# Wangshihu12/colmap-pcd

Measured on AMD Instinct MI355X. Metric: NN queries/sec + BA-iter ms, 10M-pt cloud / 1M 3D feats, higher is better.
Workload: dtype f32 (NN distances) / f64 (association, BA); 1 GPU; M: 10000000-pt 'planes' cloud / 1000000 queries + BA scene 1000 cams / 1000000 pts / 4721253 obs / 900000 lidar terms (OPENCV), the same total at every N; cloud_points=10000000, queries=1000000, queries_this_rank=1000000, parallelism=single GPU

## Files before the change

### colmap-pcd_amd/csrc/nn.hip

```cpp
#include <atomic>
#include <cfloat>

#include "cloud.h"
#include "grid.h"
#include "prim.h"
#include "scratch.h"

namespace pcd {

void free_query_scratch(QueryScratch* s) { delete s; }

constexpr uint64_t kKeyInit = (uint64_t)0x7F7FFFFFu << 32;
constexpr uint64_t kSmallBatch = 65536;

struct BrickParams {
  int B, R;
  int Bx;
  int nb[3];
  uint32_t nbricks;
};

constexpr int kBrickCells = 2, kBrickCellsX = 2, kBrickHalo = 2;

static BrickParams make_bricks(const GridParams& g) {
// ... 542 lines not shown
  const uint32_t n = *count_ptr;
  const uint32_t e0 = (blockIdx.x * kFbcThreads + tid) * kFbcPer;
  if (blockIdx.x * kFbcThreads * kFbcPer >= n) return;
  uint32_t v[kFbcPer], cnt = 0;
  if (e0 + kFbcPer <= n) {
    const uint4 q = *reinterpret_cast<const uint4*>(list + e0);
    v[0] = q.x; v[1] = q.y; v[2] = q.z; v[3] = q.w;
  } else {
#pragma unroll
    for (uint32_t k = 0; k < kFbcPer; ++k) v[k] = e0 + k < n ? list[e0 + k] : 0xFFFFFFFFu;
  }
#pragma unroll
  for (uint32_t k = 0; k < kFbcPer; ++k) cnt += v[k] != 0xFFFFFFFFu ? 1u : 0u;
  const uint32_t inc = wave_scan_add_u32(cnt);
  if (lane == 63) s_wave[wave] = inc;
  __syncthreads();
  uint32_t before = 0, total = 0;
  for (uint32_t w = 0; w < kFbcThreads / 64; ++w) { before += w < wave ? s_wave[w] : 0u; total += s_wave[w]; }
  if (tid == 0) s_base = total ? atomicAdd(dense_count, total) : 0u;
  __syncthreads();
  uint32_t pos = s_base + before + inc - cnt;
#pragma unroll
  for (uint32_t k = 0; k < kFbcPer; ++k)
    if (v[k] != 0xFFFFFFFFu) dense[pos++] = v[k];
}

struct FbFused {
  const double* q;
  const double* max_range;
  uint64_t mr_count;
  double fixed_range;
};

template <int FUSED>
__global__ __launch_bounds__(256) void k_nn_fallback(GridParams g, PyramidParams py, const float4* __restrict__ sorted,
                                                      const uint32_t* __restrict__ cell_start,
                                                      const float* __restrict__ aabb,
                                                      const float4* __restrict__ seeds,
                                                      const float4* __restrict__ qf4,
                                                      const uint32_t* __restrict__ list,
                                                      const uint32_t* __restrict__ count_ptr, uint32_t count_imm,
                                                      uint64_t* __restrict__ keys, NnCounters* __restrict__ ctr,
                                                      int collect_stats, FbFused fu) {
  constexpr int kStack = kMaxPyrLevels - 2;
  __shared__ float s_lb[4][kStack][64];
  __shared__ uint32_t s_rng[4][kStack][64];
  __shared__ unsigned long long s_mask[4][kStack];
  const int lane = threadIdx.x & 63;
  const int wave = __builtin_amdgcn_readfirstlane((int)(threadIdx.x >> 6));
  const uint32_t count = count_ptr ? *count_ptr : count_imm;
  const uint32_t nwaves = gridDim.x * 4;
  const int top = py.nlev - 1;
  unsigned long long st_pts = 0, st_q = 0, st_steps = 0, st_leaves = 0;
  uint32_t st_max_steps = 0, st_max_leaves = 0;
  for (uint32_t e = blockIdx.x * 4 + wave; e < count; e += nwaves) {
    const uint32_t qi = list ? list[e] : e;
    float qx, qy, qz;
    uint64_t best;
    if (FUSED == 0) {
      const float4 q = qf4[qi];
      if (q.w == 0.f) continue;
      qx = q.x; qy = q.y; qz = q.z;
      best = keys[qi];
    } else {
      qx = (float)fu.q[3 * (size_t)qi]; qy = (float)fu.q[3 * (size_t)qi + 1]; qz = (float)fu.q[3 * (size_t)qi + 2];
      if (!(isfinite(qx) && isfinite(qy) && isfinite(qz))) {
        if (lane == 0) keys[qi] = PCD_KEY_NONE;
        continue;
      }
      best = FUSED == 2 ? bounded_init_key(fu.max_range ? fu.max_range[fu.mr_count == 1 ? 0 : qi] : fu.fixed_range,
                                             fu.q[3 * (size_t)qi], fu.q[3 * (size_t)qi + 1], fu.q[3 * (size_t)qi + 2])
                          : kKeyInit;
    }
    {
      const int sx = cell_coord(qx, g.origin[0], g.inv_h, g.dims[0]) >> 3;
      const int sy = cell_coord(qy, g.origin[1], g.inv_h, g.dims[1]) >> 3;
      const int sz = cell_coord(qz, g.origin[2], g.inv_h, g.dims[2]) >> 3;
      const float4 sp = seeds[((size_t)sz * py.seed_dims[1] + sy) * py.seed_dims[0] + sx];
      const uint64_t sk = make_key(l2_simple3(qx, qy, qz, sp.x, sp.y, sp.z), __float_as_uint(sp.w));
      best = sk < best ? sk : best;
    }
    double lane_best = __builtin_bit_cast(double, best);
    float best_d = __uint_as_float((uint32_t)(best >> 32));
    int lev = top;
    float cur_lb;
    unsigned long long cur_m;
    uint32_t rs = 0, rn = 0;
    uint32_t q_steps = 0, q_leaves = 0;
#define PCD_FB_EXPAND(cf, cn)                                                                                         \
    {                                                                                                                 \
      const uint32_t cn_ = (cn);                                                                                      \
      const uint32_t last = cn_ ? cn_ - 1u : 0u;                   \
      const uint32_t id = (cf) + ((uint32_t)lane < last ? (uint32_t)lane : last);                                     \
      const float4 lo = *reinterpret_cast<const float4*>(aabb + 8 * (size_t)id);             \
      const float4 hi = *reinterpret_cast<const float4*>(aabb + 8 * (size_t)id + 4);       \
           \
                      \
      const float px = __builtin_amdgcn_fmed3f(qx, lo.x, lo.w), pyc = __builtin_amdgcn_fmed3f(qy, lo.y, hi.x),        \
                  pz = __builtin_amdgcn_fmed3f(qz, lo.z, hi.y);                                                       \
      const float lbv = l2_simple3(qx, qy, qz, px, pyc, pz);                                                          \
      cur_lb = (uint32_t)lane < cn_ ? lbv : INFINITY;                                                                 \
      rs = __float_as_uint(hi.z); rn = __float_as_uint(hi.w);                                                         \
      cur_m = __ballot(cur_lb <= best_d);                                                                             \
    }
    PCD_FB_EXPAND(py.root_first, py.root_count);
    while (true) {
      ++q_steps;
      unsigned long long m = cur_m & __ballot(cur_lb <= best_d);
      if (m == 0) {
        if (lev == top) break;
        ++lev;
        cur_lb = s_lb[wave][lev - 2][lane];
        const uint32_t pr = s_rng[wave][lev - 2][lane];
        rs = pr & (kMaxPyrRecords - 1u); rn = (pr >> 26) + 1u;
        const unsigned long long pm = s_mask[wave][lev - 2];
        cur_m = ((unsigned long long)(uint32_t)__builtin_amdgcn_readfirstlane((int)(pm >> 32)) << 32) |
                (uint32_t)__builtin_amdgcn_readfirstlane((int)pm);
        continue;
      }
      const int sl = wave_argmin_u32(__float_as_uint(cur_lb), m);
      m &= ~(1ull << sl);
      cur_m = m;
      if (lev == 1) {
        const uint32_t s0 = (uint32_t)__builtin_amdgcn_readlane((int)rs, sl), n0 = (uint32_t)__builtin_amdgcn_readlane((int)rn, sl);
        for (uint32_t base = 0; base < n0; base += 128) {
          float4 p[2];
#pragma unroll
          for (int k = 0; k < 2; ++k) {
            const uint32_t gi = base + k * 64 + lane;
            p[k] = sorted[s0 + (gi < n0 ? gi : n0 - 1)];
          }
#pragma unroll
          for (int k = 0; k < 2; ++k) {
            const float d = l2_simple3(qx, qy, qz, p[k].x, p[k].y, p[k].z);
            lane_best = min_key_f64(lane_best, __builtin_bit_cast(double, make_key(d, __float_as_uint(p[k].w))));
          }
        }
        st_pts += n0;
        ++q_leaves;
        best = wave_min_u64(__builtin_bit_cast(uint64_t, lane_best));
        best_d = __uint_as_float((uint32_t)(best >> 32));
        unsigned long long mb = m & __ballot(cur_lb <= best_d);
        if (mb) {
          cur_m = m & ~mb;
          while (mb) {
            uint32_t a[4], c[4];
            uint32_t cmax = 0;
#pragma unroll
            for (int k = 0; k < 4; ++k) {
              const int r = mb ? __ffsll((long long)mb) - 1 : -1;
              mb &= mb - 1;
              a[k] = r >= 0 ? (uint32_t)__builtin_amdgcn_readlane((int)rs, r) : a[0];
              c[k] = r >= 0 ? (uint32_t)__builtin_amdgcn_readlane((int)rn, r) : 0u;
              cmax = c[k] > cmax ? c[k] : cmax;
              st_pts += c[k];
              q_leaves += r >= 0 ? 1 : 0;
            }
            for (uint32_t base = 0; base < cmax; base += 64) {
              float4 p[4];
              const uint32_t gi = base + lane;
#pragma unroll
              for (int k = 0; k < 4; ++k) p[k] = sorted[a[k] + (gi < c[k] ? gi : (c[k] ? c[k] - 1 : 0u))];
#pragma unroll
              for (int k = 0; k < 4; ++k) {
                const float d = l2_simple3(qx, qy, qz, p[k].x, p[k].y, p[k].z);
                lane_best = min_key_f64(lane_best, __builtin_bit_cast(double, make_key(d, __float_as_uint(p[k].w))));
              }
            }
          }
          best = wave_min_u64(__builtin_bit_cast(uint64_t, lane_best));
          best_d = __uint_as_float((uint32_t)(best >> 32));
        }
      } else {
        s_lb[wave][lev - 2][lane] = cur_lb;
        s_rng[wave][lev - 2][lane] = rs | ((rn - 1u) << 26);
        if (lane == 0) s_mask[wave][lev - 2] = cur_m;
        const uint32_t cf = (uint32_t)__builtin_amdgcn_readlane((int)rs, sl), cn = (uint32_t)__builtin_amdgcn_readlane((int)rn, sl);
        --lev;
        PCD_FB_EXPAND(cf, cn);
      }
    }
#undef PCD_FB_EXPAND
    if (lane == 0) keys[qi] = finalized_key(best);
    st_q += 1;
    st_steps += q_steps; st_leaves += q_leaves;
    st_max_steps = q_steps > st_max_steps ? q_steps : st_max_steps;
    st_max_leaves = q_leaves > st_max_leaves ? q_leaves : st_max_leaves;
  }
  if (collect_stats) {
    __shared__ unsigned long long s_st[4];
    __shared__ unsigned int s_mx[2];
    if (threadIdx.x < 4) s_st[threadIdx.x] = 0;
    if (threadIdx.x < 2) s_mx[threadIdx.x] = 0;
    __syncthreads();
    if (lane == 0) {
      atomicAdd(&s_st[0], st_pts); atomicAdd(&s_st[1], st_q); atomicAdd(&s_st[2], st_steps); atomicAdd(&s_st[3], st_leaves);
      atomicMax(&s_mx[0], st_max_steps); atomicMax(&s_mx[1], st_max_leaves);
    }
    __syncthreads();
    if (threadIdx.x == 0 && s_st[1]) {
      atomicAdd(&ctr->fallback_points, s_st[0]);
      atomicAdd(&ctr->pair_evals, s_st[0]);
      atomicAdd(&ctr->fallback_queries, s_st[1]);
      atomicAdd(&ctr->fb_steps, s_st[2]); atomicAdd(&ctr->fb_leaves, s_st[3]);
      atomicMax(&ctr->fb_max_steps, s_mx[0]); atomicMax(&ctr->fb_max_leaves, s_mx[1]);
    }
  }
}

constexpr unsigned g_fb_max_blocks = 16384;
struct FbQueries {
  const float4* qf4;
  FbFused fused;
  const uint32_t *list, *list_count;
};
template <int FUSED>
static void launch_fallback(const pcd_cloud* c, const float4* seeds, const FbQueries& src, uint64_t n, uint64_t* keys,
                            NnCounters* ctr, int collect_stats, hipStream_t s) {
  hipLaunchKernelGGL(k_nn_fallback<FUSED>, dim3((unsigned)std::min<uint64_t>(div_up(n, 4), g_fb_max_blocks)), dim3(256), 0,
                     s, c->grid, c->pyr, c->sorted.p, c->cell_start.p, c->blk_aabb.p, seeds, src.qf4, src.list,
                     src.list_count, src.list_count ? 0u : (uint32_t)n, keys, ctr, collect_stats, src.fused);
}
static std::atomic<int> g_collect_stats{0};
#ifdef PCD_ABLATE
static const int g_brick_blocks_per_cu = std::getenv("PCD_BRICK_BLOCKS") ? std::atoi(std::getenv("PCD_BRICK_BLOCKS")) : PCD_BRICK_MINWAVES;
#else
constexpr int g_brick_blocks_per_cu = PCD_BRICK_MINWAVES;
#endif
static std::atomic<int> g_nn_kernel{0};
static std::atomic<int> g_bk_sort{0};
static std::atomic<int> g_nn_schedule{0};

static pcd_status brick_slots(pcd_cloud* c, QueryScratch* sc, const BrickParams& b, hipStream_t s) {
  if (sc->bk_slot.p && sc->bk_nslots == b.nbricks) return PCD_OK;
  PCD_TRY(sc->bk_slot.reserve((size_t)b.nbricks / 32 + 1));
  DevBuf<uint32_t> flag;
  PCD_TRY(flag.reserve((size_t)b.nbricks + 1));
  hipLaunchKernelGGL(k_brick_occupied, dim3(div_up(b.nbricks, 256)), dim3(256), 0, s, c->grid, b, c->cell_start.p, flag.p);
  hipLaunchKernelGGL(k_brick_bitmap, dim3(div_up(div_up(b.nbricks, 32), 256)), dim3(256), 0, s, flag.p, b.nbricks, sc->bk_slot.p);
  PCD_HIP_TRY(hipStreamSynchronize(s));
  sc->bk_nslots = b.nbricks;
  return PCD_OK;
}

__global__ void k_seed_init(GridParams g, int sdx, int sdy, int sdz, float4* __restrict__ seeds, float4* __restrict__ qf4,
                            uint64_t* __restrict__ keys) {
  const uint64_t i = blockIdx.x * (uint64_t)blockDim.x + threadIdx.x;
  if (i >= (uint64_t)sdx * sdy * sdz) return;
  const int x = (int)(i % sdx), y = (int)((i / sdx) % sdy), z = (int)(i / ((uint64_t)sdx * sdy));
  seeds[i] = make_float4(INFINITY, INFINITY, INFINITY, 0.f);
  const float cx = 0.5f * (float)(8 * x + min(8 * x + 8, g.dims[0])), cy = 0.5f * (float)(8 * y + min(8 * y + 8, g.dims[1])),
              cz = 0.5f * (float)(8 * z + min(8 * z + 8, g.dims[2]));
  qf4[i] = make_float4(g.origin[0] + cx * g.h, g.origin[1] + cy * g.h, g.origin[2] + cz * g.h, 1.f);
  keys[i] = kKeyInit;
}
__global__ void k_seed_gather(const uint64_t* __restrict__ keys, uint64_t n, ShardIndex si, const float4* __restrict__ pts4,
                              float4* __restrict__ seeds) {
  const uint64_t i = blockIdx.x * (uint64_t)blockDim.x + threadIdx.x;
  if (i >= n) return;
  const uint64_t k = keys[i];
  const uint64_t row = k == PCD_KEY_NONE ? ~0ull : shard_local_row(si, (uint32_t)k);
  if (row == ~0ull) return;
  const float4 p = pts4[row];
  seeds[i] = make_float4(p.x, p.y, p.z, __uint_as_float((uint32_t)k));
}
static pcd_status fb_seed_table(pcd_cloud* c, QueryScratch* sc, hipStream_t s) {
  if (sc->fb_seed_ok) return PCD_OK;
  const PyramidParams& py = c->pyr;
  const uint64_t n = (uint64_t)py.seed_dims[0] * py.seed_dims[1] * py.seed_dims[2];
  DevBuf<float4> qf4;
  DevBuf<uint64_t> keys;
  DevBuf<float4>& seeds = sc->fb_seed;
  PCD_TRY(seeds.reserve(n));
  PCD_TRY(qf4.reserve(n));
  PCD_TRY(keys.reserve(n));
  hipLaunchKernelGGL(k_seed_init, dim3(div_up(n, 256)), dim3(256), 0, s, c->grid, py.seed_dims[0], py.seed_dims[1],
                     py.seed_dims[2], seeds.p, qf4.p, keys.p);
  launch_fallback<0>(c, seeds.p, {qf4.p}, n, keys.p, nullptr, 0, s);
  hipLaunchKernelGGL(k_seed_gather, dim3(div_up(n, 256)), dim3(256), 0, s, keys.p, n, c->shard_index(), c->pts4.p, seeds.p);
  PCD_HIP_TRY(hipGetLastError());
  PCD_HIP_TRY(hipStreamSynchronize(s));
  sc->fb_seed_ok = true;
  return PCD_OK;
}

static pcd_status counters_ready(QueryScratch* sc, hipStream_t s) {
  if (sc->counters.p) return PCD_OK;
  PCD_TRY(sc->counters.reserve(2));
  PCD_HIP_TRY(hipMemsetAsync(sc->counters.p, 0, 2 * sizeof(NnCounters), s));
  sc->ctr_cur = 0;
  sc->ctr_next_clean = true;
  return PCD_OK;
}
enum class CtrUse { kAlternate, kClear, kClearForStats };
static pcd_status take_counters(QueryScratch* sc, CtrUse use, int collect_stats, hipStream_t s, NnCounters** ctr,
                                NnCounters** ctr_next = nullptr) {
  PCD_TRY(counters_ready(sc, s));
  const bool clean = use == CtrUse::kAlternate ? sc->ctr_next_clean : use == CtrUse::kClearForStats && !collect_stats;
  if (use == CtrUse::kAlternate) {
    sc->ctr_cur = 1 - sc->ctr_cur;
    sc->ctr_next_clean = false;
  }
  *ctr = sc->counters.p + sc->ctr_cur;
  if (ctr_next) *ctr_next = sc->counters.p + (1 - sc->ctr_cur);
  if (!clean) PCD_HIP_TRY(hipMemsetAsync(*ctr, 0, sizeof(NnCounters), s));
  return PCD_OK;
}
static void counters_left_clean(QueryScratch* sc) { sc->ctr_next_clean = true; }

static void launch_prepare(const NnCall& call, uint64_t Q, float4* qf4, uint64_t* d_keys, hipStream_t s) {
  ScopedKernelTimer t("nn_prepare", s);
// ... 67 lines not shown
    unsigned end_bit = 1;
    while (end_bit < 32 && ((uint64_t)1 << end_bit) <= (uint64_t)b.nbricks + 1) ++end_bit;
#ifndef PCD_SORT_MERGE_LIMIT
#define PCD_SORT_MERGE_LIMIT 262144
#endif
    using SortCfg = rocprim::radix_sort_config<rocprim::default_config, rocprim::default_config,
                                               rocprim::default_config, PCD_SORT_MERGE_LIMIT>;
    PCD_TRY(sort_pairs<SortCfg>(sc->tmp, k0, k1, v0, v1, (unsigned)Q, 0u, end_bit, s));
    const unsigned ntiles = div_up(Q, kBkTile);
    hipLaunchKernelGGL(k_brick_tile_count<kGroup>, dim3(ntiles), dim3(256), 0, s, k1, (uint32_t)Q, b.nbricks, sc->bk_item.p);
    hipLaunchKernelGGL(k_brick_emit<kGroup>, dim3(ntiles), dim3(256), 0, s, k1, v1, sc->bk_item.p, sc->qf4.p, carried_keys,
                       (uint32_t)Q, b.nbricks, (uint32_t)b.nb[0], (uint32_t)b.nb[1], sc->items.p, sc->qsorted.p,
                       sc->ksorted.p, sc->fb_list.p, ctr);
  }
  {
    ScopedKernelTimer t("nn_brick", s);
    const unsigned blocks = (unsigned)std::min<uint64_t>(div_up(div_up(Q, kGroup), 4) + 1, 256 * (uint64_t)g_brick_blocks_per_cu);
    int fl = (collect_stats & ~(2 | 4 | 8)) | (nn_kernel == 1 ? 2 : 0) | (nn_schedule == 1 ? 8 : 0);
    if ((collect_stats & 5) == 5) {
      PCD_TRY(sc->wave_rec.reserve(3 * (size_t)blocks * 4));
      sc->wave_rec_n = blocks * 4;
      fl |= 4;
    } else {
      sc->wave_rec_n = 0;
    }
    hipLaunchKernelGGL(k_nn_brick_clip, dim3(blocks), dim3(256), 0, s, g, c->sorted.p, c->cell_start.p, sc->qsorted.p,
                       sc->ksorted.p, sc->items.p, ctr, d_keys, sc->fb_list.p, &ctr->fb_count, fl, sc->wave_rec.p);
  }
  {
    ScopedKernelTimer t("nn_fallback", s);
    PCD_TRY(sc->fb_dense.reserve(Q));
    hipLaunchKernelGGL(k_fb_compact, dim3(div_up(fb_cap, kFbcThreads * kFbcPer)), dim3(kFbcThreads), 0, s, sc->fb_list.p,
                       &ctr->fb_count, sc->fb_dense.p, &ctr->pad[0]);
    launch_fallback<0>(c, sc->fb_seed.p, {sc->qf4.p, {}, sc->fb_dense.p, &ctr->pad[0]}, Q, d_keys, ctr, collect_stats, s);
  }
  PCD_HIP_TRY(hipGetLastError());
  if (counting) counters_left_clean(sc);
  return PCD_OK;
}

enum class NnPath { kEmptyCloud, kBruteForce, kOneLaunch, kPrepareWalk, kGrid };
static pcd_status choose_path(bool empty_cloud, int algo, uint64_t Q, int prep, NnPath* path) {
  const NnPath walk = prep == kPrepRefine ? NnPath::kPrepareWalk : NnPath::kOneLaunch;
  if (empty_cloud) *path = NnPath::kEmptyCloud;
  else if (algo == PCD_NN_BRUTEFORCE) *path = NnPath::kBruteForce;
  else if (algo == PCD_NN_FALLBACK_ONLY) *path = walk;
  else if (algo == PCD_NN_AUTO) *path = Q <= kSmallBatch ? walk : NnPath::kGrid;
  else if (algo == PCD_NN_GRID) *path = NnPath::kGrid;
  else {
    set_error("unknown nn algo %d", algo);
    return PCD_ERR_INVALID;
  }
  return PCD_OK;
}

static pcd_status nn_device(pcd_cloud* c, const NnCall& call, uint64_t Q, int algo, uint64_t* d_keys, hipStream_t s) {
  QueryScratch* sc = scratch_of(c);
  if (Q == 0) return PCD_OK;
  PCD_REQUIRE(Q < 0xFFFFFFF0ull, "more than 2^32 queries in one call");
  sc->wave_rec_n = 0;
  NnPath path;
  PCD_TRY(choose_path(c->m == 0, algo, Q, call.prep, &path));
  const int collect_stats = g_collect_stats.load();
  NnCounters* ctr;
  switch (path) {
    case NnPath::kEmptyCloud:
    case NnPath::kBruteForce:
      PCD_TRY(sc->qf4.reserve(Q));
      launch_prepare(call, Q, sc->qf4.p, d_keys, s);
      if (path == NnPath::kBruteForce) launch_bruteforce(c, sc->qf4.p, Q, d_keys, s);
      launch_finalize(Q, d_keys, s);
      break;
    case NnPath::kOneLaunch: {
      PCD_TRY(fb_seed_table(c, sc, s));
      PCD_TRY(take_counters(sc, CtrUse::kClearForStats, collect_stats, s, &ctr));
      ScopedKernelTimer t("nn_fallback", s);
      const FbQueries src{nullptr, FbFused{call.pa.q, call.pa.max_range, call.pa.mr_count, call.pa.fixed_range}};
      if (call.prep == kPrepBounded) launch_fallback<2>(c, sc->fb_seed.p, src, Q, d_keys, ctr, collect_stats, s);
      else launch_fallback<1>(c, sc->fb_seed.p, src, Q, d_keys, ctr, collect_stats, s);
      break;
    }
    case NnPath::kPrepareWalk: {
      PCD_TRY(fb_seed_table(c, sc, s));
      PCD_TRY(sc->qf4.reserve(Q));
      launch_prepare(call, Q, sc->qf4.p, d_keys, s);
      PCD_TRY(take_counters(sc, CtrUse::kClear, collect_stats, s, &ctr));
      ScopedKernelTimer t("nn_fallback", s);
      launch_fallback<0>(c, sc->fb_seed.p, {sc->qf4.p}, Q, d_keys, ctr, collect_stats, s);
      break;
    }
    case NnPath::kGrid:
      PCD_TRY(fb_seed_table(c, sc, s));
      PCD_TRY(sc->qf4.reserve(Q));
      PCD_TRY(run_grid(c, sc, Q, d_keys, s, call));
      break;
  }
  PCD_HIP_TRY(hipGetLastError());
  return PCD_OK;
}

static NnCall make_call(int prep, const pcd_cloud* c, const double* d_q, const uint8_t* d_skip = nullptr,
                        const double* d_max_range = nullptr, uint64_t mr_count = 0, double fixed_range = 0.0) {
  const BoxF box{c->bb_lo[0], c->bb_lo[1], c->bb_lo[2], c->bb_hi[0], c->bb_hi[1], c->bb_hi[2]};
  return {prep, {d_q, d_skip, box, d_max_range, mr_count, fixed_range}};
}

pcd_status nn_query_device_internal(pcd_cloud* c, const double* d_q, uint64_t Q, int algo, uint64_t* d_keys,
                                    hipStream_t s) {
  return nn_device(c, make_call(kPrepPlain, c, d_q), Q, algo, d_keys, s);
}
pcd_status nn_query_bounded_internal(pcd_cloud* c, const double* d_q, uint64_t Q, const double* d_max_range,
                                     uint64_t mr_count, double fixed_range, uint64_t* d_keys, hipStream_t s) {
  return nn_device(c, make_call(kPrepBounded, c, d_q, nullptr, d_max_range, mr_count, fixed_range), Q, PCD_NN_AUTO, d_keys, s);
}

}

using namespace pcd;

extern "C" {

// ... 72 lines not shown
  return PCD_OK;
}

pcd_status pcd_nn_set_schedule(int schedule) {
  if (schedule < 0) return PCD_OK;
  PCD_REQUIRE(schedule <= 1, "schedule must be 0 (static rounds + dynamic chunks) or 1 (static)");
  g_nn_schedule = schedule;
  return PCD_OK;
}

pcd_status pcd_nn_schedule_params(int* static_pct, int* chunk) {
  PCD_REQUIRE(static_pct && chunk, "null pointer");
  *static_pct = (int)kSchedStaticPct;
  *chunk = (int)kSchedChunk;
  return PCD_OK;
}

pcd_status pcd_nn_last_wave_records(pcd_cloud* c, uint64_t* records, uint64_t cap_waves, uint64_t* nwaves, uint64_t* nitems) {
  PCD_REQUIRE(c && nwaves && nitems, "null pointer");
  *nwaves = *nitems = 0;
  if (!c->scratch || !c->scratch->counters.p) return PCD_OK;
  QueryScratch* sc = c->scratch;
  PCD_HIP_TRY(hipSetDevice(c->device));
  PCD_HIP_TRY(hipDeviceSynchronize());
  NnCounters h;
  PCD_HIP_TRY(hipMemcpy(&h, sc->counters.p + sc->ctr_cur, sizeof h, hipMemcpyDeviceToHost));
  *nitems = h.nitems;
  *nwaves = sc->wave_rec_n;
  const uint64_t n = std::min<uint64_t>(cap_waves, sc->wave_rec_n);
  if (n && records) PCD_HIP_TRY(hipMemcpy(records, sc->wave_rec.p, n * 3 * sizeof(uint64_t), hipMemcpyDeviceToHost));
  return PCD_OK;
}

pcd_status pcd_nn_set_bookkeeping(int radix_sort) {
  g_bk_sort = radix_sort ? 1 : 0;
  return PCD_OK;
}

pcd_status pcd_nn_set_tuning(int brick_cells, int halo_cells, int collect_stats) {
  if ((brick_cells != 0 && brick_cells != kBrickCells) || (halo_cells >= 0 && halo_cells != kBrickHalo)) {
    set_error("pcd_nn_set_tuning: the brick geometry is fixed at %d cells with a halo of %d (asked for %d / %d)",
              kBrickCells, kBrickHalo, brick_cells, halo_cells);
    return PCD_ERR_UNSUPPORTED;
  }
#ifdef PCD_ABLATE
  g_collect_stats = collect_stats;
#else
  g_collect_stats = collect_stats & 5;
#endif
  return PCD_OK;
}

}
```

### colmap-pcd_amd/csrc/scratch.h

```cpp
#pragma once
#include <cstddef>

#include "cloud.h"

namespace pcd {

#ifndef PCD_SCHED_CURSOR_WORDS
#define PCD_SCHED_CURSOR_WORDS 32
#endif
constexpr int kSchedCursorWords = PCD_SCHED_CURSOR_WORDS;

struct alignas(128) NnCounters {
  unsigned long long brick_groups, staged_points, fallback_queries, fallback_points, pair_evals;
  unsigned int nitems, fb_count;
  unsigned int pad[2];
  unsigned int n_in_grid;
  unsigned int pad2[3];
  unsigned int fb_max_steps, fb_max_leaves;
  unsigned long long fb_steps, fb_leaves;
  alignas(128) unsigned int sched_cursor[8 * kSchedCursorWords];
};

static_assert(sizeof(NnCounters) % 128 == 0 && offsetof(NnCounters, sched_cursor) % 128 == 0, "cursors on line boundaries in both blocks");

struct QueryScratch {
  DevBuf<float4> qf4;
  DevBuf<uint64_t> keys;
  DevBuf<uint32_t> bk_keys, bk_vals;
  DevBuf<uint32_t> bk_item;
  DevBuf<uint32_t> bk_slot, bk_chist;
  DevBuf<uint32_t> bk_hmat;
  uint32_t bk_nslots = 0;
  DevBuf<float4> qsorted;
  DevBuf<uint64_t> ksorted;
  DevBuf<uint4> items;
  DevBuf<uint32_t> fb_list, fb_dense;
  DevBuf<float4> fb_seed;
  bool fb_seed_ok = false;
  DevBuf<NnCounters> counters;
  int ctr_cur = 0;
  bool ctr_next_clean = false;
  DevBuf<unsigned long long> wave_rec;
  uint32_t wave_rec_n = 0;
  DevBuf<char> tmp;
  DevBuf<double> d_q;
  DevBuf<uint32_t> d_idx; DevBuf<float> d_sq; DevBuf<uint8_t> d_found;
  DevBuf<double> a_mr, a_xyz, a_abcd, a_dist, a_angle, a_d2p;
  DevBuf<uint8_t> a_type;
  DevBuf<uint64_t> a_keys;
  PinnedBuf<double> h_q, h_mr;
  PinnedBuf<pcd_assoc_hit> h_hits;
  PinnedBuf<uint32_t> h_count;
  static constexpr int kStageChunks = 4;
  hipStream_t st_in = nullptr, st_comp = nullptr, st_out = nullptr, st_cnt = nullptr;
  hipEvent_t ev_in[kStageChunks] = {}, ev_comp[kStageChunks] = {}, ev_cnt[kStageChunks] = {};
  ~QueryScratch() {
    for (int k = 0; k < kStageChunks; ++k) {
      if (ev_in[k]) (void)hipEventDestroy(ev_in[k]);
      if (ev_comp[k]) (void)hipEventDestroy(ev_comp[k]);
      if (ev_cnt[k]) (void)hipEventDestroy(ev_cnt[k]);
    }
    if (st_in) (void)hipStreamDestroy(st_in);
    if (st_comp) (void)hipStreamDestroy(st_comp);
    if (st_out) (void)hipStreamDestroy(st_out);
    if (st_cnt) (void)hipStreamDestroy(st_cnt);
  }
  DevBuf<pcd_assoc_hit> d_hits;
  DevBuf<uint32_t> hit_pos, hit_count;
  DevBuf<uint32_t> nr_pass, nr_off;
  DevBuf<uint2> nr_items;
  DevBuf<unsigned long long> nr_part;
  DevBuf<char> nr_tmp;
  DevBuf<uint32_t> nr_count;
  DevBuf<double> nr_curv;
};

// ... 12 lines not shown
```

### colmap-pcd_amd/pcdhip/__init__.py

```python
import ctypes as C
import os
import subprocess

import numpy as np

_PKG = os.path.dirname(os.path.abspath(__file__))
_ROOT = os.path.dirname(_PKG)
LIB_PATH = os.environ.get("PCDHIP_LIB", os.path.join(_ROOT, "libpcdhip.so"))

PCD_OK, PCD_ERR_INVALID, PCD_ERR_NO_DEVICE, PCD_ERR_HIP, PCD_ERR_OOM, PCD_ERR_UNSUPPORTED = range(6)
NN_AUTO, NN_BRUTEFORCE, NN_FALLBACK_ONLY, NN_GRID = 0, 1, 2, 3
GATE_MAPPER_LOCAL, GATE_MAPPER_GLOBAL, GATE_CONTROLLER = 0, 1, 2
GATE_BOUNDED_SEARCH = 0x100
LIDAR_NONE, LIDAR_ICP, LIDAR_ICP_GROUND = 0, 1, 2
LIDAR_PROJ = 3
LOSS_TRIVIAL, LOSS_SOFT_L1, LOSS_CAUCHY = 0, 1, 2
LAYOUT_XYZ_NRM, LAYOUT_AOS32 = 0, 1
NORMALS_ORIENT_NONE, NORMALS_ORIENT_VIEWPOINT = 0, 1
KEY_NONE = 0x7FFFFFFFFFFFFFFF

CAMERA_MODELS = ["SIMPLE_PINHOLE", "PINHOLE", "SIMPLE_RADIAL", "RADIAL", "OPENCV", "OPENCV_FISHEYE",
                 "FULL_OPENCV", "FOV", "SIMPLE_RADIAL_FISHEYE", "RADIAL_FISHEYE", "THIN_PRISM_FISHEYE"]


# ... 309 lines not shown
    if not os.path.exists(LIB_PATH):
        raise PcdError(PCD_ERR_NO_DEVICE, f"{LIB_PATH} not built; run __graft_entry__.build() or make -C colmap-pcd_amd")
    if os.environ.get("PCDHIP_NO_TORCH_PRELOAD", "0") != "1":
        try:
            import torch
        except ImportError:
            pass
    L = C.CDLL(LIB_PATH)
    L.pcd_last_error.restype = C.c_char_p
    L.pcd_cloud_size.restype = C.c_uint64
    L.pcd_cloud_size.argtypes = [C.c_void_p]
    L.pcd_cloud_create.argtypes = [C.c_void_p, C.c_void_p, C.c_uint64, C.POINTER(CloudOptions), C.POINTER(C.c_void_p)]
    L.pcd_cloud_destroy.argtypes = [C.c_void_p]
    L.pcd_cloud_destroy.restype = None
    L.pcd_cloud_get_info.argtypes = [C.c_void_p, C.POINTER(CloudInfo)]
    L.pcd_cloud_download.argtypes = [C.c_void_p, C.c_void_p, C.c_void_p]
    L.pcd_nn_query_algo.argtypes = [C.c_void_p, C.c_void_p, C.c_uint64, C.c_int, C.c_void_p, C.c_void_p, C.c_void_p]
    L.pcd_nn_query.argtypes = [C.c_void_p, C.c_void_p, C.c_uint64, C.c_void_p, C.c_void_p, C.c_void_p]
    L.pcd_nn_query_device.argtypes = [C.c_void_p, C.c_void_p, C.c_uint64, C.c_int, C.c_void_p, C.c_void_p]
    L.pcd_associate.argtypes = [C.c_void_p, C.c_void_p, C.c_uint64, C.c_void_p, C.c_uint64, C.c_int,
                                C.POINTER(AssocOut)]
    L.pcd_associate_device.argtypes = [C.c_void_p, C.c_void_p, C.c_uint64, C.c_void_p, C.c_uint64, C.c_int,
                                       C.c_void_p, C.POINTER(AssocOut), C.c_void_p]
    L.pcd_nn_winner_payload_device.argtypes = [C.c_void_p, C.c_void_p, C.c_uint64, C.c_void_p, C.c_void_p]
    L.pcd_associate_from_payload_device.argtypes = [C.c_int, C.c_void_p, C.c_uint64, C.c_void_p, C.c_uint64,
                                                    C.c_int, C.c_void_p, C.c_void_p, C.POINTER(AssocOut),
                                                    C.c_void_p]
    L.pcd_search_range_schedule.argtypes = [C.c_void_p, C.c_uint64, C.c_double, C.c_double, C.c_double, C.c_void_p]
    L.pcd_profile_get.argtypes = [C.POINTER(KernelTime), C.c_int, C.POINTER(C.c_int)]
    L.pcd_nn_last_stats.argtypes = [C.c_void_p, C.POINTER(NNStats)]
    if hasattr(L, "pcd_nn_last_wave_records"):
        L.pcd_nn_last_wave_records.argtypes = [C.c_void_p, C.c_void_p, C.c_uint64, C.POINTER(C.c_uint64),
                                               C.POINTER(C.c_uint64)]
    L.pcd_normals_options_default.argtypes = [C.POINTER(NormalsOptions)]
    L.pcd_normals_options_default.restype = None
    L.pcd_cloud_estimate_normals_device.argtypes = [C.c_void_p, C.POINTER(NormalsOptions), C.c_void_p, C.c_void_p,
                                                    C.c_void_p]
    L.pcd_cloud_estimate_normals.argtypes = [C.c_void_p, C.POINTER(NormalsOptions), C.c_void_p, C.c_void_p,
                                             C.POINTER(NormalsInfo)]
    L.pcd_voxel_options_default.argtypes = [C.POINTER(VoxelOptions)]
    L.pcd_voxel_options_default.restype = None
    L.pcd_cloud_voxel_downsample.argtypes = [C.c_void_p, C.POINTER(VoxelOptions), C.c_void_p, C.POINTER(C.c_void_p),
                                             C.POINTER(VoxelInfo)]
    L.pcd_cloud_voxel_downsample_device.argtypes = [C.c_void_p, C.POINTER(VoxelOptions), C.c_void_p, C.c_void_p,
                                                    C.POINTER(C.c_void_p), C.POINTER(VoxelInfo)]
    if hasattr(L, "pcd_ba_create"):
        L.pcd_ba_create.argtypes = [C.POINTER(BADesc), C.POINTER(C.c_void_p)]
        L.pcd_ba_destroy.argtypes = [C.c_void_p]
        L.pcd_ba_destroy.restype = None
        L.pcd_ba_set_parameters.argtypes = [C.c_void_p, C.c_void_p, C.c_void_p]
        L.pcd_ba_evaluate.argtypes = [C.c_void_p, C.POINTER(BAOut)]
        L.pcd_ba_evaluate_device.argtypes = [C.c_void_p, C.POINTER(BAOut), C.c_void_p]
        L.pcd_ba_device_parameters.argtypes = [C.c_void_p, C.POINTER(C.c_void_p), C.POINTER(C.c_void_p)]
        L.pcd_ba_set_camera_parameters.argtypes = [C.c_void_p, C.c_void_p]
        L.pcd_ba_evaluate_blocks.argtypes = [C.c_void_p, C.c_int, C.c_int, C.POINTER(BABlocks)]
        L.pcd_ba_evaluate_blocks_compact.argtypes = [C.c_void_p, C.c_int, C.c_int, C.POINTER(BABlocksCompact)]
    if hasattr(L, "pcd_ba_schur_device"):
        L.pcd_ba_set_parameters_device.argtypes = [C.c_void_p, C.c_void_p, C.c_void_p, C.c_void_p]
        L.pcd_ba_schur_structure.argtypes = [C.c_void_p, C.c_void_p, C.POINTER(C.c_int32), C.POINTER(C.c_uint64),
                                             C.c_void_p, C.c_void_p]
        L.pcd_ba_schur_device.argtypes = [C.c_void_p, C.POINTER(BASchurOpts), C.POINTER(BASchurOut), C.c_void_p]
        L.pcd_ba_schur.argtypes = [C.c_void_p, C.POINTER(BASchurOpts), C.POINTER(BASchurOut)]
        L.pcd_ba_schur_back_substitute_device.argtypes = [C.c_void_p, C.c_void_p, C.c_void_p, C.c_void_p, C.c_void_p]
        L.pcd_ba_plus_device.argtypes = [C.c_void_p] + [C.c_void_p] * 5
        L.pcd_ba_schur_stats.argtypes = [C.c_void_p, C.POINTER(BASchurInfo)]
    if hasattr(L, "pcd_ba_solve"):
# ... 242 lines not shown
        L = lib()
        L.pcd_associate_staged.argtypes = [C.c_void_p, C.c_uint64, C.c_uint64, C.c_int, C.POINTER(C.c_void_p),
                                           C.POINTER(C.c_uint64)]
        h, n = C.c_void_p(), C.c_uint64(0)
        _check(L.pcd_associate_staged(self._h, Q, mr_count, gate_mode, C.byref(h), C.byref(n)))
        if n.value == 0:
            return np.zeros(0, HIT_DTYPE)
        buf = (C.c_char * (80 * n.value)).from_address(h.value)
        return np.frombuffer(buf, dtype=HIT_DTYPE, count=n.value)

    def associate_device(self, d_q, Q, d_max_range, mr_count, gate_mode, d_out, d_keys_in=None, stream=0):
        ao = AssocOut(*[_ptr(d_out.get(k)) for k in ("lidar_xyz", "abcd", "type", "dist", "angle", "dist2plane",
                                                      "nn_idx", "nn_sqdist")])
        _check(lib().pcd_associate_device(self._h, _ptr(d_q), Q, _ptr(d_max_range), mr_count, gate_mode,
                                          _ptr(d_keys_in), C.byref(ao), C.c_void_p(stream)))

    def winner_payload_device(self, d_keys, Q, d_payload, stream=0):
        _check(lib().pcd_nn_winner_payload_device(self._h, _ptr(d_keys), Q, _ptr(d_payload), C.c_void_p(stream)))

    def last_stats(self):
        s = NNStats()
        _check(lib().pcd_nn_last_stats(self._h, C.byref(s)))
        return {n: getattr(s, n) for n, _ in NNStats._fields_}

    def last_wave_records(self):
        L = lib()
        nw, ni = C.c_uint64(0), C.c_uint64(0)
        _check(L.pcd_nn_last_wave_records(self._h, None, 0, C.byref(nw), C.byref(ni)))
        rec = np.zeros((nw.value, 3), np.uint64)
        if nw.value:
            _check(L.pcd_nn_last_wave_records(self._h, _vp(rec), nw.value, C.byref(nw), C.byref(ni)))
        return rec, int(ni.value)


def associate_from_payload_device(device, d_q, Q, d_max_range, mr_count, gate_mode, d_keys, d_payload, d_out,
                                  stream=0):
    ao = AssocOut(*[_ptr(d_out.get(k)) for k in ("lidar_xyz", "abcd", "type", "dist", "angle", "dist2plane",
                                                  "nn_idx", "nn_sqdist")])
    _check(lib().pcd_associate_from_payload_device(device, _ptr(d_q), Q, _ptr(d_max_range), mr_count, gate_mode,
                                                   _ptr(d_keys), _ptr(d_payload), C.byref(ao), C.c_void_p(stream)))


class ShardReduce(C.Structure):
    MINFN = C.CFUNCTYPE(C.c_int, C.c_void_p, C.POINTER(C.c_void_p), C.POINTER(C.c_int), C.c_int, C.c_uint64)
    SUMFN = C.CFUNCTYPE(C.c_int, C.c_void_p, C.POINTER(C.c_void_p), C.POINTER(C.c_int), C.c_int, C.c_uint64)
    _fields_ = [("min_u64", MINFN), ("sum_i32", SUMFN), ("user", C.c_void_p)]


class _BorrowedCloud(Cloud):

    def __init__(self, handle, owner):
        self._h = C.c_void_p(handle)
        self._owner = owner
        self.device = 0

    def close(self):
        self._h = None


class ShardedCloud:

    def __init__(self, xyz, nrm, devices, raw_lidar_frame=True, cell_size=0.0, layout=LAYOUT_XYZ_NRM):
        L = lib()
        xyz = np.ascontiguousarray(xyz, np.float32)
        if layout == LAYOUT_AOS32:
            xyz, nrm = xyz.reshape(-1, 8), None
# ... 1188 lines not shown
```

Measured before the change: 879.8 million queries/s.

## Run NN fallback as one wave per block with dynamic LDS stack

Changes the fallback tree-walk kernel from 256-thread blocks (four waves sharing static LDS sized for the deepest pyramid) to 64-thread single-wave blocks. Each block now gets a dynamically sized LDS stack matched to the actual pyramid depth, the SGPR budget is capped, and the block limit is raised. The block-level stats reduction with its __syncthreads is replaced by per-wave atomics, which lets waves retire independently. It also adds an optional per-wave timing probe buffer and a host API to read it; the per-wave atomics could add contention when stats are on.

```diff
diff --git a/colmap-pcd_amd/csrc/nn.hip b/colmap-pcd_amd/csrc/nn.hip
--- a/colmap-pcd_amd/csrc/nn.hip
+++ b/colmap-pcd_amd/csrc/nn.hip
@@ -598,28 +598,30 @@
   double fixed_range;
 };
 
+constexpr size_t fb_stack_bytes(int nlev) { return (size_t)(nlev - 2) * (64 * 4 + 64 * 4 + 8); }
+static_assert(fb_stack_bytes(kMaxPyrLevels) <= 64 * 1024, "the deepest pyramid's stack fits a workgroup's LDS");
 template <int FUSED>
-__global__ __launch_bounds__(256) void k_nn_fallback(GridParams g, PyramidParams py, const float4* __restrict__ sorted,
-                                                      const uint32_t* __restrict__ cell_start,
-                                                      const float* __restrict__ aabb,
-                                                      const float4* __restrict__ seeds,
-                                                      const float4* __restrict__ qf4,
-                                                      const uint32_t* __restrict__ list,
-                                                      const uint32_t* __restrict__ count_ptr, uint32_t count_imm,
-                                                      uint64_t* __restrict__ keys, NnCounters* __restrict__ ctr,
-                                                      int collect_stats, FbFused fu) {
-  constexpr int kStack = kMaxPyrLevels - 2;
-  __shared__ float s_lb[4][kStack][64];
-  __shared__ uint32_t s_rng[4][kStack][64];
-  __shared__ unsigned long long s_mask[4][kStack];
-  const int lane = threadIdx.x & 63;
-  const int wave = __builtin_amdgcn_readfirstlane((int)(threadIdx.x >> 6));
+__global__ __launch_bounds__(64) __attribute__((amdgpu_num_sgpr(80)))
+void k_nn_fallback(GridParams g, PyramidParams py, const float4* __restrict__ sorted,
+                   const uint32_t* __restrict__ cell_start, const float* __restrict__ aabb,
+                   const float4* __restrict__ seeds, const float4* __restrict__ qf4,
+                   const uint32_t* __restrict__ list,
+                   const uint32_t* __restrict__ count_ptr, uint32_t count_imm, uint64_t* __restrict__ keys,
+                   NnCounters* __restrict__ ctr, int collect_stats, FbFused fu,
+                   unsigned long long* __restrict__ wave_rec) {
+  extern __shared__ __attribute__((aligned(16))) unsigned char s_stack[];
+  const int lane = threadIdx.x;
+  const int nst = py.nlev - 2;
+  float* const s_lb = reinterpret_cast<float*>(s_stack);
+  uint32_t* const s_rng = reinterpret_cast<uint32_t*>(s_stack) + (size_t)nst * 64;
+  unsigned long long* const s_mask = reinterpret_cast<unsigned long long*>(s_stack + (size_t)nst * 512);
   const uint32_t count = count_ptr ? *count_ptr : count_imm;
-  const uint32_t nwaves = gridDim.x * 4;
   const int top = py.nlev - 1;
+  const bool probe = (collect_stats & 16) != 0;
+  const unsigned long long t_start = probe ? wall_clock64() : 0ull;
   unsigned long long st_pts = 0, st_q = 0, st_steps = 0, st_leaves = 0;
   uint32_t st_max_steps = 0, st_max_leaves = 0;
-  for (uint32_t e = blockIdx.x * 4 + wave; e < count; e += nwaves) {
+  for (uint32_t e = blockIdx.x; e < count; e += gridDim.x) {
     const uint32_t qi = list ? list[e] : e;
     float qx, qy, qz;
     uint64_t best;
@@ -676,10 +678,10 @@
       if (m == 0) {
         if (lev == top) break;
         ++lev;
-        cur_lb = s_lb[wave][lev - 2][lane];
-        const uint32_t pr = s_rng[wave][lev - 2][lane];
+        cur_lb = s_lb[(lev - 2) * 64 + lane];
+        const uint32_t pr = s_rng[(lev - 2) * 64 + lane];
         rs = pr & (kMaxPyrRecords - 1u); rn = (pr >> 26) + 1u;
-        const unsigned long long pm = s_mask[wave][lev - 2];
+        const unsigned long long pm = s_mask[lev - 2];
         cur_m = ((unsigned long long)(uint32_t)__builtin_amdgcn_readfirstlane((int)(pm >> 32)) << 32) |
                 (uint32_t)__builtin_amdgcn_readfirstlane((int)pm);
         continue;
@@ -738,9 +740,9 @@
           best_d = __uint_as_float((uint32_t)(best >> 32));
         }
       } else {
-        s_lb[wave][lev - 2][lane] = cur_lb;
-        s_rng[wave][lev - 2][lane] = rs | ((rn - 1u) << 26);
-        if (lane == 0) s_mask[wave][lev - 2] = cur_m;
+        s_lb[(lev - 2) * 64 + lane] = cur_lb;
+        s_rng[(lev - 2) * 64 + lane] = rs | ((rn - 1u) << 26);
+        if (lane == 0) s_mask[lev - 2] = cur_m;
         const uint32_t cf = (uint32_t)__builtin_amdgcn_readlane((int)rs, sl), cn = (uint32_t)__builtin_amdgcn_readlane((int)rn, sl);
         --lev;
         PCD_FB_EXPAND(cf, cn);
@@ -753,39 +755,38 @@
     st_max_steps = q_steps > st_max_steps ? q_steps : st_max_steps;
     st_max_leaves = q_leaves > st_max_leaves ? q_leaves : st_max_leaves;
   }
-  if (collect_stats) {
-    __shared__ unsigned long long s_st[4];
-    __shared__ unsigned int s_mx[2];
-    if (threadIdx.x < 4) s_st[threadIdx.x] = 0;
-    if (threadIdx.x < 2) s_mx[threadIdx.x] = 0;
-    __syncthreads();
-    if (lane == 0) {
-      atomicAdd(&s_st[0], st_pts); atomicAdd(&s_st[1], st_q); atomicAdd(&s_st[2], st_steps); atomicAdd(&s_st[3], st_leaves);
-      atomicMax(&s_mx[0], st_max_steps); atomicMax(&s_mx[1], st_max_leaves);
-    }
-    __syncthreads();
-    if (threadIdx.x == 0 && s_st[1]) {
-      atomicAdd(&ctr->fallback_points, s_st[0]);
-      atomicAdd(&ctr->pair_evals, s_st[0]);
-      atomicAdd(&ctr->fallback_queries, s_st[1]);
-      atomicAdd(&ctr->fb_steps, s_st[2]); atomicAdd(&ctr->fb_leaves, s_st[3]);
-      atomicMax(&ctr->fb_max_steps, s_mx[0]); atomicMax(&ctr->fb_max_leaves, s_mx[1]);
-    }
-  }
-}
-
-constexpr unsigned g_fb_max_blocks = 16384;
+  if (probe && lane == 0) {
+    unsigned long long* const rec = wave_rec + 3u * blockIdx.x;
+    rec[0] = t_start; rec[1] = wall_clock64(); rec[2] = st_steps;
+  }
+  if ((collect_stats & 1) && lane == 0 && st_q) {
+    atomicAdd(&ctr->fallback_points, st_pts);
+    atomicAdd(&ctr->pair_evals, st_pts);
+    atomicAdd(&ctr->fallback_queries, st_q);
+    atomicAdd(&ctr->fb_steps, st_steps); atomicAdd(&ctr->fb_leaves, st_leaves);
+    atomicMax(&ctr->fb_max_steps, st_max_steps); atomicMax(&ctr->fb_max_leaves, st_max_leaves);
+  }
+}
+
+constexpr unsigned g_fb_max_blocks = 65536;
 struct FbQueries {
   const float4* qf4;
   FbFused fused;
   const uint32_t *list, *list_count;
 };
 template <int FUSED>
-static void launch_fallback(const pcd_cloud* c, const float4* seeds, const FbQueries& src, uint64_t n, uint64_t* keys,
-                            NnCounters* ctr, int collect_stats, hipStream_t s) {
-  hipLaunchKernelGGL(k_nn_fallback<FUSED>, dim3((unsigned)std::min<uint64_t>(div_up(n, 4), g_fb_max_blocks)), dim3(256), 0,
+static pcd_status launch_fallback(const pcd_cloud* c, const float4* seeds, const FbQueries& src, uint64_t n, uint64_t* keys,
+                                  NnCounters* ctr, int collect_stats, hipStream_t s) {
+  const unsigned blocks = (unsigned)std::min<uint64_t>(n, g_fb_max_blocks);
+  QueryScratch* sc = c->scratch;
+  if (collect_stats & 16) {
+    PCD_TRY(sc->fb_rec.reserve(3 * (size_t)blocks));
+    sc->fb_rec_n = blocks;
+  }
+  hipLaunchKernelGGL(k_nn_fallback<FUSED>, dim3(blocks), dim3(64), fb_stack_bytes(c->pyr.nlev),
                      s, c->grid, c->pyr, c->sorted.p, c->cell_start.p, c->blk_aabb.p, seeds, src.qf4, src.list,
-                     src.list_count, src.list_count ? 0u : (uint32_t)n, keys, ctr, collect_stats, src.fused);
+                     src.list_count, src.list_count ? 0u : (uint32_t)n, keys, ctr, collect_stats, src.fused, sc->fb_rec.p);
+  return PCD_OK;
 }
 static std::atomic<int> g_collect_stats{0};
 #ifdef PCD_ABLATE
@@ -842,7 +843,7 @@
   PCD_TRY(keys.reserve(n));
   hipLaunchKernelGGL(k_seed_init, dim3(div_up(n, 256)), dim3(256), 0, s, c->grid, py.seed_dims[0], py.seed_dims[1],
                      py.seed_dims[2], seeds.p, qf4.p, keys.p);
-  launch_fallback<0>(c, seeds.p, {qf4.p}, n, keys.p, nullptr, 0, s);
+  PCD_TRY(launch_fallback<0>(c, seeds.p, {qf4.p}, n, keys.p, nullptr, 0, s));
   hipLaunchKernelGGL(k_seed_gather, dim3(div_up(n, 256)), dim3(256), 0, s, keys.p, n, c->shard_index(), c->pts4.p, seeds.p);
   PCD_HIP_TRY(hipGetLastError());
   PCD_HIP_TRY(hipStreamSynchronize(s));
@@ -976,7 +977,7 @@
     PCD_TRY(sc->fb_dense.reserve(Q));
     hipLaunchKernelGGL(k_fb_compact, dim3(div_up(fb_cap, kFbcThreads * kFbcPer)), dim3(kFbcThreads), 0, s, sc->fb_list.p,
                        &ctr->fb_count, sc->fb_dense.p, &ctr->pad[0]);
-    launch_fallback<0>(c, sc->fb_seed.p, {sc->qf4.p, {}, sc->fb_dense.p, &ctr->pad[0]}, Q, d_keys, ctr, collect_stats, s);
+    PCD_TRY(launch_fallback<0>(c, sc->fb_seed.p, {sc->qf4.p, {}, sc->fb_dense.p, &ctr->pad[0]}, Q, d_keys, ctr, collect_stats, s));
   }
   PCD_HIP_TRY(hipGetLastError());
   if (counting) counters_left_clean(sc);
@@ -1002,7 +1003,7 @@
   QueryScratch* sc = scratch_of(c);
   if (Q == 0) return PCD_OK;
   PCD_REQUIRE(Q < 0xFFFFFFF0ull, "more than 2^32 queries in one call");
-  sc->wave_rec_n = 0;
+  sc->wave_rec_n = sc->fb_rec_n = 0;
   NnPath path;
   PCD_TRY(choose_path(c->m == 0, algo, Q, call.prep, &path));
   const int collect_stats = g_collect_stats.load();
@@ -1020,8 +1021,8 @@
       PCD_TRY(take_counters(sc, CtrUse::kClearForStats, collect_stats, s, &ctr));
       ScopedKernelTimer t("nn_fallback", s);
       const FbQueries src{nullptr, FbFused{call.pa.q, call.pa.max_range, call.pa.mr_count, call.pa.fixed_range}};
-      if (call.prep == kPrepBounded) launch_fallback<2>(c, sc->fb_seed.p, src, Q, d_keys, ctr, collect_stats, s);
-      else launch_fallback<1>(c, sc->fb_seed.p, src, Q, d_keys, ctr, collect_stats, s);
+      if (call.prep == kPrepBounded) PCD_TRY(launch_fallback<2>(c, sc->fb_seed.p, src, Q, d_keys, ctr, collect_stats, s));
+      else PCD_TRY(launch_fallback<1>(c, sc->fb_seed.p, src, Q, d_keys, ctr, collect_stats, s));
       break;
     }
     case NnPath::kPrepareWalk: {
@@ -1030,7 +1031,7 @@
       launch_prepare(call, Q, sc->qf4.p, d_keys, s);
       PCD_TRY(take_counters(sc, CtrUse::kClear, collect_stats, s, &ctr));
       ScopedKernelTimer t("nn_fallback", s);
-      launch_fallback<0>(c, sc->fb_seed.p, {sc->qf4.p}, Q, d_keys, ctr, collect_stats, s);
+      PCD_TRY(launch_fallback<0>(c, sc->fb_seed.p, {sc->qf4.p}, Q, d_keys, ctr, collect_stats, s));
       break;
     }
     case NnPath::kGrid:
@@ -1169,6 +1170,21 @@
   return PCD_OK;
 }
 
+pcd_status pcd_nn_last_fb_wave_records(pcd_cloud* c, uint64_t* records, uint64_t cap_waves, uint64_t* nwaves,
+                                       uint64_t* waves_per_block) {
+  PCD_REQUIRE(c && nwaves && waves_per_block, "null pointer");
+  *nwaves = 0;
+  *waves_per_block = 1;
+  if (!c->scratch) return PCD_OK;
+  QueryScratch* sc = c->scratch;
+  PCD_HIP_TRY(hipSetDevice(c->device));
+  PCD_HIP_TRY(hipDeviceSynchronize());
+  *nwaves = sc->fb_rec_n;
+  const uint64_t n = std::min<uint64_t>(cap_waves, sc->fb_rec_n);
+  if (n && records) PCD_HIP_TRY(hipMemcpy(records, sc->fb_rec.p, n * 3 * sizeof(uint64_t), hipMemcpyDeviceToHost));
+  return PCD_OK;
+}
+
 pcd_status pcd_nn_set_bookkeeping(int radix_sort) {
   g_bk_sort = radix_sort ? 1 : 0;
   return PCD_OK;
@@ -1183,7 +1199,7 @@
 #ifdef PCD_ABLATE
   g_collect_stats = collect_stats;
 #else
-  g_collect_stats = collect_stats & 5;
+  g_collect_stats = collect_stats & 21;
 #endif
   return PCD_OK;
 }
diff --git a/colmap-pcd_amd/csrc/scratch.h b/colmap-pcd_amd/csrc/scratch.h
--- a/colmap-pcd_amd/csrc/scratch.h
+++ b/colmap-pcd_amd/csrc/scratch.h
@@ -42,6 +42,8 @@
   bool ctr_next_clean = false;
   DevBuf<unsigned long long> wave_rec;
   uint32_t wave_rec_n = 0;
+  DevBuf<unsigned long long> fb_rec;
+  uint32_t fb_rec_n = 0;
   DevBuf<char> tmp;
   DevBuf<double> d_q;
   DevBuf<uint32_t> d_idx; DevBuf<float> d_sq; DevBuf<uint8_t> d_found;
diff --git a/colmap-pcd_amd/pcdhip/__init__.py b/colmap-pcd_amd/pcdhip/__init__.py
--- a/colmap-pcd_amd/pcdhip/__init__.py
+++ b/colmap-pcd_amd/pcdhip/__init__.py
@@ -365,6 +365,9 @@
     if hasattr(L, "pcd_nn_last_wave_records"):
         L.pcd_nn_last_wave_records.argtypes = [C.c_void_p, C.c_void_p, C.c_uint64, C.POINTER(C.c_uint64),
                                                C.POINTER(C.c_uint64)]
+    if hasattr(L, "pcd_nn_last_fb_wave_records"):
+        L.pcd_nn_last_fb_wave_records.argtypes = [C.c_void_p, C.c_void_p, C.c_uint64, C.POINTER(C.c_uint64),
+                                                  C.POINTER(C.c_uint64)]
     L.pcd_normals_options_default.argtypes = [C.POINTER(NormalsOptions)]
     L.pcd_normals_options_default.restype = None
     L.pcd_cloud_estimate_normals_device.argtypes = [C.c_void_p, C.POINTER(NormalsOptions), C.c_void_p, C.c_void_p,
@@ -673,6 +676,15 @@
             _check(L.pcd_nn_last_wave_records(self._h, _vp(rec), nw.value, C.byref(nw), C.byref(ni)))
         return rec, int(ni.value)
 
+    def last_fb_wave_records(self):
+        L = lib()
+        nw, wpb = C.c_uint64(0), C.c_uint64(0)
+        _check(L.pcd_nn_last_fb_wave_records(self._h, None, 0, C.byref(nw), C.byref(wpb)))
+        rec = np.zeros((nw.value, 3), np.uint64)
+        if nw.value:
+            _check(L.pcd_nn_last_fb_wave_records(self._h, _vp(rec), nw.value, C.byref(nw), C.byref(wpb)))
+        return rec, int(wpb.value)
+
 
 def associate_from_payload_device(device, d_q, Q, d_max_range, mr_count, gate_mode, d_keys, d_payload, d_out,
                                   stream=0):
```

Measured after the change: 897.2 million queries/s (median of 6 runs). 1.02x the previous value.
